# andrewjong/SwapNet

Hardware: AMD Instinct MI355X
Metric: images/sec full G+D step, warp-stage 256x256 bs=32/GPU (higher is better)
Workload: dtype f32; 1 GPU; warp-stage G+D optimize_parameters step, 256x256, bs 32/GPU, fp32 storage and accumulation, GEMM products on the 16-bit MFMA pipe from operand splits: forward / input-gradient GEMMs as 2 fp16 planes of amax-scaled operands (22 of 24 mantissa bits, 3 of 4 terms, the dropped one below 2^-22), weight-gradient GEMMs in the same two-plane form, train mode (dropout 0.5), WarpModule 137.6M + PatchGAN 2.8; step_form=eager launches, global_batch=32, parallelism=dp1

## Files before the change

### include/swapnet_hip.h

```cpp
#ifndef SWAPNET_HIP_H
#define SWAPNET_HIP_H

#include <stddef.h>
#include <stdint.h>

#ifdef __cplusplus
extern "C" {
#endif

typedef struct swn_ctx swn_ctx;
typedef struct swn_model swn_model;

int swn_abi_version(void);
const char* swn_last_error(void);
int swn_is_device_build(void);

int swn_ctx_create(int device, void* hip_stream, int create_stream, size_t workspace_bytes, swn_ctx** out);
int swn_ctx_destroy(swn_ctx* ctx);
int swn_ctx_set_overlap(swn_ctx* ctx, int on);
int swn_ctx_set_patchgan_layers(swn_ctx* ctx, int n_layers);
int swn_ctx_set_patchgan_norm(swn_ctx* ctx, int kind);
int swn_ctx_sync(swn_ctx* ctx);
int swn_ctx_bytes_allocated(swn_ctx* ctx, size_t* out);

int swn_prof_enable(int on);
int swn_prof_reset(void);
int swn_prof_report(char* buf, int len);
int swn_probe_mfma(swn_ctx* ctx, int zeros, int iters, float* out4);
int swn_route_trace(int on);
int swn_route_report(char* buf, int len);
int swn_slot_audit(int on);

int swn_warp_model_create(swn_ctx* ctx, int batch, int height, int width, int is_train, float dropout,
                          swn_model** out);
int swn_texture_model_create(swn_ctx* ctx, int batch, int height, int width, int is_train, int num_roi,
// ... 84 lines not shown
int swn_model_weight_arena(swn_model* m, int net, float** dev_ptr, size_t* count);
int swn_model_arena(swn_model* m, int net, int which, float** dev_ptr, size_t* count);

int swn_op_roi_align(swn_ctx* ctx, const float* tex, int b, int c, int h, int w, const float* rois, int r,
                     int ph, int pw, float* out);
int swn_op_roi_align_indices(swn_ctx* ctx, const float* rois, int k, int h, int w, int ph, int pw, int32_t* idx,
                             uint8_t* valid);
int swn_op_decode_labels(swn_ctx* ctx, const float* x, int b, int c, int h, int w, uint8_t* rgb);
int swn_op_argmax_labels(swn_ctx* ctx, const float* x, int b, int c, int h, int w, int32_t* labels);
int swn_op_labels_to_onehot(swn_ctx* ctx, const int32_t* labels, int b, int c, int h, int w, float* out);
int swn_op_conv(swn_ctx* ctx, int kind, int transposed, int what, int naive, float* x, int n, int ci, int h, int w,
                float* wgt, int co, const float* bias, int act, float* y);
int swn_op_conv_produced(swn_ctx* ctx, int kind, int transposed, int what, int naive, float* x, int n, int ci, int h, int w,
                         float* wgt, int co, const float* bias, int act, float* y, int pre, int post, float* x_out, float* x_slot,
                         float* y_slot, float* z_slot, float* dy_out, float* dy_slot, int* kscale_out);
int swn_op_instance_norm_act(swn_ctx* ctx, const float* x, int n, int c, int h, int w, int act, float* y);
int swn_op_instance_norm_act_bwd(swn_ctx* ctx, const float* x, const float* dy, int n, int c, int h, int w, int act,
                                 float* dx);
int swn_op_batch_norm_act(swn_ctx* ctx, const float* x, int n, int c, int h, int w, int groups, int act, int training,
                          const float* weight, const float* bias, float* running_mean, float* running_var,
                          int64_t* num_batches_tracked, float* y, float* save_stats);
int swn_op_batch_norm_act_bwd(swn_ctx* ctx, const float* x, const float* dy, int n, int c, int h, int w, int groups, int act,
                              const float* weight, const float* bias, float* dx, float* dweight, float* dbias);
int swn_op_batch_norm_act_dropout(swn_ctx* ctx, const float* x, const float* dy, int n, int c, int h, int w, int act, float p,
                                  uint64_t seed, const float* weight, const float* bias, float* y, float* mask, float* dx,
                                  float* dweight, float* dbias);
int swn_op_norm_act_time(swn_ctx* ctx, int kind, int what, const float* x, const float* dy, int n, int c, int h, int w, int groups,
                         int act, int warmup, int iters, float* ms_out);
int swn_op_affine_gather(swn_ctx* ctx, const float* src, float* dst, int b, int c, int h, int w, const double* maps,
                         int nmaps);
// ... 37 lines not shown
```

### swapnet_amd/_C.py

```python
import ctypes as C
import os

_HERE = os.path.dirname(os.path.abspath(__file__))
LIB_PATH = os.path.join(_HERE, "csrc", "libswapnet_hip.so")

LOSS_NAMES = ("D", "D_real", "D_fake", "G", "G_gan", "G_ce", "G_l1", "G_content", "G_style", "D_gp")


class SwnHyper(C.Structure):
    _fields_ = [(n, C.c_float) for n in ("lr", "d_lr", "weight_decay", "d_weight_decay", "b1", "b2",
                                         "lambda_gan", "lambda_ce", "lambda_l1", "lambda_content",
                                         "lambda_style")] + [("gan_mode", C.c_int), ("warp_mode_ce", C.c_int), ("grad_scale", C.c_float),
                                                                           ("d_b1", C.c_float), ("d_b2", C.c_float),
                                                                           ("gp_mode", C.c_int), ("lambda_gp", C.c_float)]


class SwapnetHipError(RuntimeError):
    pass


_vp, _fp, _i, _f = C.c_void_p, C.c_void_p, C.c_int, C.c_float

_PROTOS = {
    "swn_abi_version": ([], _i),
    "swn_is_device_build": ([], _i),
    "swn_ctx_create": ([_i, _vp, _i, C.c_size_t, C.POINTER(_vp)], _i),
    "swn_ctx_destroy": ([_vp], _i),
    "swn_ctx_sync": ([_vp], _i),
    "swn_ctx_set_overlap": ([_vp, _i], _i),
    "swn_ctx_set_patchgan_layers": ([_vp, _i], _i),
    "swn_ctx_set_patchgan_norm": ([_vp, _i], _i),
    "swn_ctx_bytes_allocated": ([_vp, C.POINTER(C.c_size_t)], _i),
    "swn_prof_enable": ([_i], _i),
    "swn_prof_reset": ([], _i),
    "swn_prof_report": ([C.c_char_p, _i], _i),
    "swn_probe_mfma": ([_vp, _i, _i, C.POINTER(C.c_float)], _i),
    "swn_route_trace": ([_i], _i),
    "swn_route_report": ([C.c_char_p, _i], _i),
    "swn_slot_audit": ([_i], _i),
    "swn_warp_model_create": ([_vp, _i, _i, _i, _i, _f, C.POINTER(_vp)], _i),
    "swn_texture_model_create": ([_vp, _i, _i, _i, _i, _i, C.POINTER(_vp)], _i),
    "swn_warp_model_create_ex": ([_vp, _i, _i, _i, _i, _f, _i, _i, C.POINTER(_vp)], _i),
    "swn_texture_model_create_ex": ([_vp, _i, _i, _i, _i, _i, _i, C.POINTER(_vp)], _i),
    "swn_texture_model_create_netG": ([_vp, _i, _i, _i, _i, _i, _i, _i, C.POINTER(_vp)], _i),
    "swn_model_create_shared": ([_vp, _i, _i, _i, C.POINTER(_vp)], _i),
# ... 42 lines not shown
    "swn_model_step": ([_vp, C.POINTER(_f * 3), _i, C.c_uint64], _i),
    "swn_model_step_captured": ([_vp, C.POINTER(_f * 3), _i, C.c_uint64], _i),
    "swn_model_step_dp": ([_vp, C.POINTER(_f * 3), _i, C.c_uint64, _i], _i),
    "swn_ctx_attach_comm": ([_vp, _vp, _vp, _i], _i),
    "swn_model_get_losses": ([_vp, C.POINTER(_f), _i], _i),
    "swn_model_grad_arena": ([_vp, _i, C.POINTER(_vp), C.POINTER(C.c_size_t)], _i),
    "swn_model_weight_arena": ([_vp, _i, C.POINTER(_vp), C.POINTER(C.c_size_t)], _i),
    "swn_model_arena": ([_vp, _i, _i, C.POINTER(_vp), C.POINTER(C.c_size_t)], _i),
    "swn_op_roi_align": ([_vp, _fp, _i, _i, _i, _i, _fp, _i, _i, _i, _fp], _i),
    "swn_op_roi_align_indices": ([_vp, _fp, _i, _i, _i, _i, _i, _vp, _vp], _i),
    "swn_op_decode_labels": ([_vp, _fp, _i, _i, _i, _i, _vp], _i),
    "swn_op_argmax_labels": ([_vp, _fp, _i, _i, _i, _i, _vp], _i),
    "swn_op_labels_to_onehot": ([_vp, _vp, _i, _i, _i, _i, _fp], _i),
    "swn_op_conv": ([_vp, _i, _i, _i, _i, _fp, _i, _i, _i, _i, _fp, _i, _fp, _i, _fp], _i),
    "swn_op_conv_produced": ([_vp, _i, _i, _i, _i, _fp, _i, _i, _i, _i, _fp, _i, _fp, _i, _fp, _i, _i, _fp, _fp, _fp, _fp, _fp, _fp, _vp], _i),
    "swn_op_instance_norm_act": ([_vp, _fp, _i, _i, _i, _i, _i, _fp], _i),
    "swn_op_instance_norm_act_bwd": ([_vp, _fp, _fp, _i, _i, _i, _i, _i, _fp], _i),
    "swn_op_batch_norm_act": ([_vp, _fp, _i, _i, _i, _i, _i, _i, _i, _fp, _fp, _fp, _fp, _vp, _fp, _fp], _i),
    "swn_op_batch_norm_act_bwd": ([_vp, _fp, _fp, _i, _i, _i, _i, _i, _i, _fp, _fp, _fp, _fp, _fp], _i),
    "swn_op_batch_norm_act_dropout": ([_vp, _fp, _fp, _i, _i, _i, _i, _i, _f, C.c_uint64, _fp, _fp, _fp, _fp, _fp, _fp, _fp], _i),
    "swn_op_norm_act_time": ([_vp, _i, _i, _fp, _fp, _i, _i, _i, _i, _i, _i, _i, _i, C.POINTER(C.c_float)], _i),
    "swn_op_affine_gather": ([_vp, _fp, _fp, _i, _i, _i, _i, _vp, _i], _i),
    "swn_op_texture_batch": ([_vp, _vp, _i, _i, _i, _vp, _i, _i, _fp, _i, _fp, C.POINTER(_f), C.POINTER(_f), _i, _i, _i, _i, _i,
                             _fp, _fp, _fp, _fp], _i),
    "swn_op_resize_u8": ([_vp, _vp, C.c_size_t, _vp, _i, _i, _i, _vp], _i),
    "swn_op_warp_batch": ([_vp, _vp, _i, _i, _i, _vp, _vp, _i, _i, _vp, _i, C.POINTER(_f), C.POINTER(_f), _i, _i, _i, _i, _i, _i,
                          _fp, _fp, _fp], _i),
    "swn_op_gan_loss": ([_vp, _i, _fp, _i, _i, _i, _i, _f, _i, _f, _fp, _fp], _i),
    "swn_op_loss": ([_vp, _i, _fp, _fp, _i, _i, _i, _i, _i, _f, _i, _i, _i, _fp, _fp, _fp], _i),
    "swn_op_bias_grad": ([_vp, _fp, _i, _i, _i, _i, _i, _fp], _i),
# ... 67 lines not shown
```

### swapnet_amd/csrc/capi.cpp

```cpp
#include <algorithm>
#include <cstring>
#include <memory>
#include <string>
#include <vector>

#include "../../include/swapnet_hip.h"
#include <cstdlib>

#include "engine.h"

using namespace swn;

struct CtxBox {
  std::unique_ptr<Ctx> c;
  void* owned_stream = nullptr;
  ~CtxBox() { c.reset(); if (owned_stream) stream_destroy(owned_stream); }
};
struct swn_ctx {
  std::shared_ptr<CtxBox> box;
  Ctx* c = nullptr;
};
struct swn_model {
  std::shared_ptr<CtxBox> keep;
  std::shared_ptr<Model> sharer;
// ... 71 lines not shown
    ctx->c->attach_comm(reinterpret_cast<Ctx::AllReduceFn>(fn), comm, fn ? world_size : 1);
  });
}
int swn_ctx_set_patchgan_layers(swn_ctx* ctx, int n_layers) {
  return guard([&] {
    REQUIRE(ctx, "ctx is NULL");
    REQUIRE(n_layers >= 0 && n_layers <= 5, "n_layers_D must be in [1, 5], or 0 for the 1x1 PixelDiscriminator");
    ctx->c->patchgan_layers = n_layers;
  });
}
int swn_ctx_set_patchgan_norm(swn_ctx* ctx, int kind) {
  return guard([&] {
    REQUIRE(ctx, "ctx is NULL");
    REQUIRE(kind >= 0 && kind <= 2, "normalization layer is not found (0 instance, 1 batch, 2 none)");
    ctx->c->patchgan_norm = kind;
  });
}
int swn_ctx_sync(swn_ctx* ctx) {
  return guard([&] { REQUIRE(ctx, "ctx is NULL"); stream_sync(ctx->c->s); });
}
int swn_ctx_bytes_allocated(swn_ctx* ctx, size_t* out) {
  return guard([&] { REQUIRE(ctx && out, "NULL argument"); *out = ctx->c->bytes_allocated; });
}

int swn_prof_enable(int on) { return guard([&] { prof_enable(on); }); }
int swn_prof_reset(void) { return guard([&] { prof_reset(); }); }
int swn_prof_report(char* buf, int len) { return prof_report(buf, len); }
int swn_probe_mfma(swn_ctx* ctx, int zeros, int iters, float* out4) {
  return guard([&] {
    REQUIRE(ctx && out4, "swn_probe_mfma: NULL argument");
// ... 618 lines not shown
        unpack_weight(s, wd.ws, A.g + wd.off, wgt);
      } else {
        A.version += 1;
        net.refresh_dgrad();
        net.backward(false, true);
        nhwc_to_nchw(s, xv.g, x, ci);
      }
      if (dy_out) nhwc_to_nchw(s, yv.g, dy_out, co);
      copy_slot(dy_slot, yv.gbase, "y.g");
    }
    if (kscale_out && net.kscale_n) dev_copy(s, kscale_out, net.kscale, std::min<size_t>(net.kscale_n, 8) * sizeof(int));
    stream_sync(s);
  });
}

int swn_op_instance_norm_act(swn_ctx* ctx, const float* x, int n, int c, int h, int w, int act, float* y) {
  return guard([&] {
    REQUIRE(ctx && x && y && c % 4 == 0, "bad argument (C must be a multiple of 4)");
    Ctx tmp(ctx->c->s);
    ParamArena A; Net net(tmp, A);
    Var xv = net.alloc_var(n, h, w, c, true), yv = net.alloc_var(n, h, w, c, true);
    net.norm_act(xv, yv, true, act, 0.f);
    net.finalize({});
    nchw_to_nhwc(tmp.s, x, n, c, h, w, xv.v);
    net.forward();
    nhwc_to_nchw(tmp.s, yv.v, y, c);
    stream_sync(tmp.s);
  });
}
int swn_op_instance_norm_act_bwd(swn_ctx* ctx, const float* x, const float* dy, int n, int c, int h, int w, int act,
// ... 511 lines not shown
```

### swapnet_amd/csrc/engine.cpp

```cpp
#include "engine.h"
#include <memory>

#include <algorithm>
#include <cstddef>
#include <cstdlib>
#include <cstring>
#include <map>
#include <string>
#include <vector>

namespace swn {

namespace {
int g_route = 0;
std::string g_route_label = "-";
char g_route_phase = '-';
std::vector<std::string> g_route_lines;
std::map<std::string, int> g_route_seen;
}
void route_enable(int on) {
  g_route = on;
  if (on) { g_route_lines.clear(); g_route_seen.clear(); g_route_label = "-"; g_route_phase = '-'; }
}
bool route_on() { return g_route != 0; }
void route_label(const char* label, char phase) { g_route_label = label ? label : "-"; g_route_phase = phase; }
void route_note(const char* kernel) {
  if (!g_route) return;
  std::string line = g_route_label + " " + std::string(1, g_route_phase) + " " + kernel;
  if (g_route_seen.emplace(line, 1).second) g_route_lines.push_back(line);
}
namespace { int g_slot_audit = 0; }
void slot_audit(int on) { g_slot_audit = on; }
bool slot_audit_on() { return g_slot_audit != 0; }

int route_report(char* buf, int len) {
  std::string out;
  for (auto& l : g_route_lines) { out += l; out += "\n"; }
  if (buf && len > 0) { strncpy(buf, out.c_str(), len - 1); buf[len - 1] = 0; }
  return (int)out.size();
}

Ctx::Ctx(void* stream, size_t ws_bytes) {
  s.handle = stream;
  s.ws_bytes = ws_bytes;
  s.ws = static_cast<char*>(dev_alloc(ws_bytes));
}
Ctx::Ctx(const Stream& shared) : s(shared), owns_ws(false) {}
Ctx::~Ctx() {
  try {
    if (owned_comm_stream) stream_sync(comm_stream);
    if (has_side) stream_sync(side);
  } catch (...) {}
  release(allocs);
  if (owns_ws) dev_free(s.ws);
// ... 528 lines not shown
  const bool wslots = wm != 2;
  const size_t slV = wslots ? reserve_slot() : 0, slD = wslots ? reserve_slot() : 0, slX = wslots ? reserve_slot() : 0;
  const bool wgrad_pairs = wslots && conv_wgrad_takes_pairs(wT, Cip, Cop);
  const bool pairV_ok = wslots && wino_fwd_takes_pairs(Cip, Cop) && (!y.has_grad || wgrad_pairs);
  const bool pairD_ok = wslots && wgrad_pairs && (!(wadj && x.has_grad && y.has_grad) || wino_fwd_takes_pairs(Cop, Cip));
  const bool pairX_ok = wslots && wino_fwd_takes_pairs(Cop, Cip);
  const size_t kV = wslots ? reserve_k() : 0, kD = wslots ? reserve_k() : 0, kX = wslots ? reserve_k() : 0;
  float* keepdM = (wadj && y.has_grad && x.has_grad && share_dy()) ? static_cast<float*>(ctx.alloc((size_t)wP * wT * Cop * sizeof(float))) : nullptr;
  const size_t pcw_off = pcw ? reserve_dgp(pcw_bs * wP) : 0, uf_off = pcw ? 0 : reserve_dg(self, (size_t)wP * Cip * Cop);
  wsV_need = std::max(wsV_need, std::max((size_t)wP * wT * std::max(Cip, Cop), (size_t)wP * wT2 * Cop));
  wsM_need = std::max(wsM_need, std::max((size_t)wP * wT * std::max(Cip, Cop), (size_t)wP * wT2 * Cip));
  wsU_need = std::max(wsU_need, (size_t)wP * Cip * Cop);
  const bool y_folds = actf != ACT_NONE && actf != ACT_TANH && wm != 2;
  const size_t ySlot = note_writer(y.vbase, y_folds);
  const float* xbase = x.vbase;
  op.fwd = [=](Net& n) {
    n.need(self);
    float* V = keepV ? keepV : n.wsV;
    const float* xin = pairV_ok ? n.slot_if_complete(xbase) : nullptr;
    wino_input_transform(n.ctx.s, wm, wr, xv, 1, gf.pad_mode, wTh, wTw, V, wslots ? n.amax + slV : nullptr, xin, n.kscale + kV);
    conv_fwd(n.ctx.s, plane_gemm(V, n.wsM, wT, Cip, Cop, Co, wP, plane_scale(xin != nullptr, n.kscale + kV, wslots ? n.amax + slV : nullptr),
                                 {pcw ? nullptr : n.dg + uf_off, n.dgp + pcw_off, pcw, pcw_bs}));
    wino_output_transform(n.ctx.s, wm, wr, n.wsM, Cop, wTh, wTw, bi >= 0 ? A->w + A->params[bi].off : nullptr, actf, yv, Co, 0,
                          y_folds ? n.amax + ySlot : nullptr);
  };

  Var scratch;
  if (y.has_grad && actf != ACT_NONE) scratch = alloc_var(yv.N, yv.H, yv.W, Cop, false);
  const bool want_dx = x.has_grad && y.has_grad;
  const int pcwt = (want_dx && wm != 2) ? wino_precut_tile(Cop, Cip) : 0;
  const size_t pcwt_bs = pcwt ? conv_precut_elems(Cop, Cip, pcwt) : 0;
  size_t pcwt_off = 0, ub_off = 0;
  if (want_dx) {
    if (pcwt) pcwt_off = reserve_dgp(pcwt_bs * wP);
    else ub_off = reserve_dg(self, (size_t)wP * Cop * Cip);
    op.grad_targets.push_back(x);
  }
// ... 360 lines not shown
  const uint64_t salt = ops.size() + 1;
  if (drop_p > 0.f) drop_sites.push_back({salt, raw.v.N, raw.v.H, raw.v.W, raw.v.C, drop_p});
  if (residual && actf != ACT_NONE) throw Error(1, "norm_act: an activation in front of a residual add is not supported");
  note_act(actf, y.v);
  const TView rv = raw.v, rg = raw.g, yv = y.v, yg = y.g;
  const size_t ySlot = note_writer(y.vbase, true);
  const size_t gSlot = (y.has_grad && raw.has_grad) ? note_writer(raw.gbase, true) : 0;
  const bool has_res = residual != nullptr;
  const Var res = has_res ? *residual : Var();
  const double* partial_in = nullptr;
  int partial_chunks = 0;
  if (norm && raw.v.H * raw.v.W > 1024 && raw.v.p == raw.vbase) {
    auto it = conv_stats.find(raw.vbase);
    if (it != conv_stats.end()) { *it->second.use = true; partial_in = it->second.partial; partial_chunks = it->second.chunks; }
  }
  op->fwd = [=](Net& n) {
    NormActArgs a;
    a.x = rv; a.y = yv; a.stats = stats; a.norm = norm; a.act = actf;
    a.partial_in = partial_in; a.partial_chunks = partial_chunks;
    a.drop_p = n.training ? drop_p : 0.f; a.seed = Net::drop_seed(n.seed, salt);
    a.seed_base = n.seed_dev; a.salt = salt;
    a.residual = has_res ? &res.v : nullptr;
    a.amax_out = n.amax + ySlot;
    norm_act_fwd(n.ctx.s, a);
  };
  if (has_res && res.has_grad && y.has_grad) op->grad_targets.push_back(res);
  const bool do_bwd = y.has_grad && raw.has_grad;
  double* colsum = nullptr;
  if (do_bwd && norm && norm_act_bwd_emits_colsum(raw.v.H * raw.v.W, raw.v.C) && raw.g.cs == raw.g.C) {
    colsum = static_cast<double*>(ctx.alloc((size_t)raw.v.N * raw.v.C * sizeof(double)));
    colsums[raw.g.p] = {colsum, raw.v.N};
// ... 779 lines not shown
```

### swapnet_amd/csrc/engine.h

```cpp
#pragma once
#include <cstdlib>
#include <functional>
#include <map>
#include <memory>
#include <string>
#include <vector>

#include "ops.h"

namespace swn {

struct Ctx {
  Stream s;
  Stream side;
  bool has_side = false, side_dirty = false;
  bool side_enabled = true;
  bool use_side() const { return has_side && side_enabled; }
  std::vector<void*> fork_events;
  size_t fork_i = 0;
  void* join_event = nullptr;
  void* owned_side_stream = nullptr;
  void enable_side(int device);
  Stream& fork_side();
  void join_side();
// ... 7 lines not shown
  void* comm_handle = nullptr;
  int comm_world = 1;
  int device_index = 0;
  Stream comm_stream;
  void* owned_comm_stream = nullptr;
  std::vector<void*> comm_events;
  size_t comm_ev_i = 0;
  void* comm_join_event = nullptr;
  bool comm_dirty = false;
  void attach_comm(AllReduceFn fn, void* comm, int world);
  Stream& comm_fork();
  void comm_join();
  void all_reduce_sum(Stream& on, float* buf, size_t count);
  int patchgan_layers = 3;
  int patchgan_norm = 0;
  explicit Ctx(void* stream, size_t ws_bytes);
  explicit Ctx(const Stream& shared);
  bool owns_ws = true;
  ~Ctx();
  void* alloc(size_t bytes);
  Ctx(const Ctx&) = delete;
  Ctx& operator=(const Ctx&) = delete;
};

struct AllocScope {
  Ctx& c; Ctx::AllocList* prev;
  AllocScope(Ctx& ctx, Ctx::AllocList& list) : c(ctx), prev(ctx.sink) { c.sink = &list; }
  ~AllocScope() { c.sink = prev; }
  AllocScope(const AllocScope&) = delete;
  AllocScope& operator=(const AllocScope&) = delete;
// ... 76 lines not shown
  int* kscale = nullptr;
  size_t kscale_n = 0;
  size_t reserve_k() { return kscale_n++; }
  struct BufSlot { size_t off = 0; bool complete = true; };
  std::map<const float*, BufSlot> buf_slots;
  std::map<const float*, const float*> ext_slots;
  size_t note_writer(const float* base, bool folds) {
    auto it = buf_slots.find(base);
    if (it == buf_slots.end()) it = buf_slots.emplace(base, BufSlot{reserve_slot(), true}).first;
    if (!folds) it->second.complete = false;
    else fold_writer_ops.push_back(ops.size());
    return it->second.off;
  }
  struct StatLink { double* partial = nullptr; int chunks = 0; std::shared_ptr<bool> use; };
  std::map<const float*, StatLink> conv_stats;
  std::vector<size_t> fold_writer_ops;
  void set_external_slot(const float* base, const float* slot) { ext_slots[base] = slot; }
  const float* slot_if_complete(const float* base) const {
    auto e = ext_slots.find(base);
    auto it = buf_slots.find(base);
    if (e != ext_slots.end()) return (it == buf_slots.end()) ? e->second : nullptr;
    if (it == buf_slots.end() || !it->second.complete || !amax) return nullptr;
    return amax + it->second.off;
  }
  bool share_dy() const;
  int dg_version = 0;
  bool keep_wino_inputs = false;
  bool s2_wino = true;
  size_t wsV_need = 0, wsM_need = 0, wsU_need = 0;
  float *wsV = nullptr, *wsM = nullptr, *wsU = nullptr;
// ... 254 lines not shown
```

### swapnet_amd/csrc/ops.h

```cpp
#pragma once
#include "common.h"
#include <cmath>
#include <cstdlib>
#include <functional>

namespace swn {

struct WShape;

inline bool env_on(const char* v) { return !(v && atoi(v) == 0); }
inline int env_int(const char* v, int dflt) { return v ? atoi(v) : dflt; }

struct Stream {
  void* handle = nullptr;
  char* ws = nullptr;
  size_t ws_bytes = 0;
};

void* event_create();
void event_destroy(void* ev);
void event_record(void* ev, Stream& s);
void stream_wait_event(Stream& s, void* ev);

void* stream_create_current();
// ... 90 lines not shown
void bias_grad(Stream& s, const TView& dy, float* db);

void reflect_fold(Stream& s, const TView& dxpad, const TView& dx, int accumulate);

void wino_input_transform(Stream& s, int m, int r, const TView& x, int pad, int pad_mode, int Th, int Tw, float* V,
                          float* amax_out = nullptr, const float* in_amax = nullptr, int* kscale_out = nullptr);
void wino_filter_transform(Stream& s, int m, int r, const WShape& w, int mode, const float* packed, float* U);
void wino_filter_transform_pc(Stream& s, int m, int r, const WShape& w, int mode, const float* packed, int bn, uint16_t* out,
                              size_t panel_elems, const float** amax_io = nullptr);
void wino_input_adjoint(Stream& s, int m, int r, float* dV, int C, int pad, int pad_mode, int Th, int Tw, const TView& dx,
                        int accumulate);
void wino_output_transform(Stream& s, int m, int r, const float* M, int Cm, int Th, int Tw, const float* bias, int act,
                           const TView& y, int Cout, int accumulate, float* amax_out = nullptr);
void wino_dy_transform(Stream& s, int m, int r, const TView& dy, int Th, int Tw, float* dM, float* amax_out = nullptr,
                       const float* in_amax = nullptr, int* kscale_out = nullptr);
void tailw_filter_transform(Stream& s, const WShape& w, const float* folded, float* U);
void tailw_filter_grad(Stream& s, const WShape& w, const float* dU, float* dfolded);
void tailw_output_transform(Stream& s, const float* M, int Th, int Tw, int Npad, const float* bias, int act, const TView& y, int Cout);
void tailw_dy_transform(Stream& s, const TView& dy, int Th, int Tw, int Npad, float* dM, float* amax_out = nullptr,
                        const float* in_amax = nullptr, int* kscale_out = nullptr);
void wino_s2_input_transform(Stream& s, const TView& fine, int Th, int Tw, float* V, float* amax_out = nullptr,
                             const float* in_amax = nullptr, int* kscale_out = nullptr);
void wino_s2_input_adjoint(Stream& s, float* dV, int Cf, int Th, int Tw, const TView& fine, const float* bias, int accumulate);
void wino_s2_filter_transform(Stream& s, const WShape& w, int mode, const float* packed, float* U);
void wino_s2_filter_grad(Stream& s, const WShape& w, const float* dU, float* dpacked);
void wino_filter_grad(Stream& s, int m, int r, const WShape& w, const float* dU, float* dpacked);

struct NormActArgs {
  TView x;
  TView y;
// ... 258 lines not shown
```

### swapnet_amd/csrc/wino.hip

```cpp
#include "hip_util.h"

namespace swn {
namespace {

__device__ __forceinline__ float4 f4add(float4 a, float4 b) { return make_float4(a.x + b.x, a.y + b.y, a.z + b.z, a.w + b.w); }
__device__ __forceinline__ float4 f4sub(float4 a, float4 b) { return make_float4(a.x - b.x, a.y - b.y, a.z - b.z, a.w - b.w); }

__device__ __forceinline__ int wsrc(int e, int ext, int pad_mode) {
  if (pad_mode == PAD_REFLECT) {
    if (e < 0) e = -e;
    else if (e >= ext) e = 2 * ext - 2 - e;
    return e;
  }
  return (e < 0 || e >= ext) ? -1 : e;
}

__global__ __launch_bounds__(256) void wino_input_kernel(const float* x, int xcs, int N, int H, int W, int C, int pad,
                                                         int pad_mode, int Th, int Tw, float* V) {
  const int C4 = C >> 2;
  const size_t T = (size_t)N * Th * Tw;
  const size_t total = T * C4;
  for (size_t i = (size_t)blockIdx.x * 256 + threadIdx.x; i < total; i += (size_t)gridDim.x * 256) {
    const size_t tile = i / C4;
    const int c = (int)(i - tile * C4) * 4;
// ... 1020 lines not shown
    }
#pragma unroll
    for (int p = 0; p < A; ++p)
#pragma unroll
      for (int j = 0; j < A; ++j) {
        float4 s = F4ZERO;
#pragma unroll
        for (int jj = 0; jj < M; ++jj) f4mac(s, F43::AT[jj][j], rr[p][jj]);
        *reinterpret_cast<float4*>(dM + ((size_t)(p * A + j) * T + tile) * CM + ph * Npad + c) = pair ? pair4(s, psc) : s;
        am = fmaxf(am, f4amax(s));
      }
  }
  if (!pair) amax_fold(am, amax_out);
}

inline unsigned wgrid(size_t total) { return (unsigned)std::min<size_t>(std::max<size_t>((total + 255) / 256, 1), 256 * 32); }

}

static int variant(int m, int r) {
  if (m == 2 && r == 3) return 0;
  if (m == 4 && r == 3) return 1;
  if (m == 3 && r == 4) return 2;
  if (m == 4 && r == 2) return 3;
  throw Error(1, "winograd: supported forms are F(2,3), F(4,3), F(3,4) and the strided F(4,2)");
}
static constexpr int wino_vec_width() { return 2; }
static float input_gain(int v) { return v == 3 ? 9.f : 100.f; }
static float dy_gain(int v) { return v == 1 ? 225.f : (v == 2 ? 49.f : 16.f); }
void wino_input_transform(Stream& s, int m, int r, const TView& x, int pad, int pad_mode, int Th, int Tw, float* V, float* amax_out,
// ... 56 lines not shown
  const dim3 grid(wgrid(total));
  if (v == 0)
    hipLaunchKernelGGL(wino_output_kernel, grid, dim3(256), 0, hs(s), M, Cm, y.N, Th, Tw, bias, act, y.p, y.cs, y.H, y.W,
                       Cout, accumulate);
  else if (v == 1)
    hipLaunchKernelGGL(winog_output_kernel<F43>, grid, dim3(256), 0, hs(s), M, Cm, y.N, Th, Tw, bias, act, y.p, y.cs, y.H,
                       y.W, Cout, accumulate, amax_out);
  else if (v == 2)
    hipLaunchKernelGGL(winog_output_kernel<F34>, grid, dim3(256), 0, hs(s), M, Cm, y.N, Th, Tw, bias, act, y.p, y.cs, y.H,
                       y.W, Cout, accumulate, amax_out);
  else
    hipLaunchKernelGGL(winog_output_kernel<F42>, grid, dim3(256), 0, hs(s), M, Cm, y.N, Th, Tw, bias, act, y.p, y.cs, y.H,
                       y.W, Cout, accumulate, amax_out);
  check_launch("wino_output_transform");
}
void wino_dy_transform(Stream& s, int m, int r, const TView& dy, int Th, int Tw, float* dM, float* amax_out, const float* in_amax,
                       int* kscale_out) {
  const int v = variant(m, r);
  if (dy.C % 4 || dy.cs % 4) throw Error(1, "wino_dy_transform: C must be a multiple of 4");
  const int vw = v == 0 ? 4 : wino_vec_width();
  const size_t total = (size_t)dy.N * Th * Tw * (dy.C / vw);
  const dim3 grid(wgrid(total));
  if (v == 0 && in_amax) throw Error(1, "wino_dy_transform: F(2,3) planes have no pair form");
#define SWN_WDY_LAUNCH(F, VW)                                                                                                       \
  hipLaunchKernelGGL((winog_dy_kernel<F, VW>), grid, dim3(256), 0, hs(s), dy.p, dy.cs, dy.N, dy.H, dy.W, dy.C, Th, Tw, dM, amax_out, \
                     in_amax, dy_gain(v), kscale_out)
  if (v == 0)
    hipLaunchKernelGGL(wino_dy_kernel, grid, dim3(256), 0, hs(s), dy.p, dy.cs, dy.N, dy.H, dy.W, dy.C, Th, Tw, dM);
  else if (v == 1) SWN_WDY_LAUNCH(F43, 2);
  else if (v == 2) SWN_WDY_LAUNCH(F34, 2);
// ... 101 lines not shown
```

### swapnet_amd/engine.py

```python
import ctypes as C
import os
from collections import OrderedDict

import torch

from . import _C

NET_G, NET_D, NET_VGG = 0, 1, 2
OPT_ADAMW, OPT_ADABOUND = 0, 1
W_WEIGHT, W_GRAD, W_EXP_AVG, W_EXP_AVG_SQ = 0, 1, 2, 3
NORM_KINDS = {"instance": 0, "batch": 1, "none": 2}
NETG_KINDS = {"swapnet": 0, "unet_128": 1}


class Context:

    def __init__(self, device=None, lib=None, workspace_mb=512, use_torch_stream=True):
        self.lib = lib or _C.lib()
        if self.lib.is_device:
            if not torch.cuda.is_available():
                raise _C.SwapnetHipError("no HIP device visible; swapnet_amd has no CPU path")
            self.device = torch.device("cuda", torch.cuda.current_device() if device is None else int(device))
            torch.cuda.set_device(self.device)
            self.torch_stream = torch.cuda.current_stream(self.device)
# ... 36 lines not shown
            cs.wait_event(st["events"][i])
        with torch.cuda.stream(cs):
            buf.copy_(t, non_blocking=True)
        main.wait_stream(cs)
        return buf, (key, i)

    def consumed(self, token):
        if token is None:
            return
        ev = torch.cuda.Event()
        ev.record(torch.cuda.current_stream(self.device))
        self._staging[token[0]]["events"][token[1]] = ev

    def set_overlap(self, on):
        self.lib.call("swn_ctx_set_overlap", self.handle, int(bool(on)))

    def sync(self):
        self.lib.call("swn_ctx_sync", self.handle)

    def attach_comm(self, fn_ptr, comm, world):
        self.lib.call("swn_ctx_attach_comm", self.handle, C.c_void_p(fn_ptr) if fn_ptr else None,
                      comm if comm is not None else None, int(world))

    def route_trace(self, on):
        self.lib.call("swn_route_trace", int(bool(on)))

    def route_report(self):
        need = self.lib.dll.swn_route_report(None, 0)
        buf = C.create_string_buffer(need + 16)
        self.lib.dll.swn_route_report(buf, need + 16)
# ... 766 lines not shown
```

Before: 1342 images/sec.

## Fuse Winograd output transform, instance norm, and next input transform in resblocks

Adds a fused kernel for small (≤16x16) resblock feature maps. One launch does the F(4,3) Winograd output transform, instance-norm statistics, activation, dropout, residual add, and the next conv's Winograd input transform, keeping the tile in shared memory. The graph builder links producer conv → norm → consumer conv through chain links so the separate output-transform, norm and input-transform launches are skipped. This cuts launches and global-memory round trips on the bottleneck layers. The costs are a statically derived amax bound for the pair-scale, low parallelism (grid C/32 × N), and order-sensitive mutable flags in the closures.

Result: no change. 1356 images/sec (median of 6 runs) (+1.0%).

```diff
diff --git a/include/swapnet_hip.h b/include/swapnet_hip.h
--- a/include/swapnet_hip.h
+++ b/include/swapnet_hip.h
@@ -19,6 +19,7 @@
 int swn_ctx_destroy(swn_ctx* ctx);
 int swn_ctx_set_overlap(swn_ctx* ctx, int on);
 int swn_ctx_set_patchgan_layers(swn_ctx* ctx, int n_layers);
+int swn_ctx_set_resblock_chain(swn_ctx* ctx, int on);
 int swn_ctx_set_patchgan_norm(swn_ctx* ctx, int kind);
 int swn_ctx_sync(swn_ctx* ctx);
 int swn_ctx_bytes_allocated(swn_ctx* ctx, size_t* out);
@@ -133,6 +134,9 @@
 int swn_op_conv_produced(swn_ctx* ctx, int kind, int transposed, int what, int naive, float* x, int n, int ci, int h, int w,
                          float* wgt, int co, const float* bias, int act, float* y, int pre, int post, float* x_out, float* x_slot,
                          float* y_slot, float* z_slot, float* dy_out, float* dy_slot, int* kscale_out);
+int swn_op_res_chain(swn_ctx* ctx, const float* x0, int n, int c, int h, int w, const float* w1, const float* b1, const float* w2,
+                     const float* b2, const float* w3, const float* b3, float drop_p, int use_residual, int keep_v, uint64_t seed,
+                     float* raw1, float* h_out, float* raw2, float* rn, float* out, float* stats1, float* stats2, int* kscale_out);
 int swn_op_instance_norm_act(swn_ctx* ctx, const float* x, int n, int c, int h, int w, int act, float* y);
 int swn_op_instance_norm_act_bwd(swn_ctx* ctx, const float* x, const float* dy, int n, int c, int h, int w, int act,
                                  float* dx);
diff --git a/swapnet_amd/_C.py b/swapnet_amd/_C.py
--- a/swapnet_amd/_C.py
+++ b/swapnet_amd/_C.py
@@ -29,6 +29,7 @@
     "swn_ctx_sync": ([_vp], _i),
     "swn_ctx_set_overlap": ([_vp, _i], _i),
     "swn_ctx_set_patchgan_layers": ([_vp, _i], _i),
+    "swn_ctx_set_resblock_chain": ([_vp, _i], _i),
     "swn_ctx_set_patchgan_norm": ([_vp, _i], _i),
     "swn_ctx_bytes_allocated": ([_vp, C.POINTER(C.c_size_t)], _i),
     "swn_prof_enable": ([_i], _i),
@@ -101,6 +102,7 @@
     "swn_op_labels_to_onehot": ([_vp, _vp, _i, _i, _i, _i, _fp], _i),
     "swn_op_conv": ([_vp, _i, _i, _i, _i, _fp, _i, _i, _i, _i, _fp, _i, _fp, _i, _fp], _i),
     "swn_op_conv_produced": ([_vp, _i, _i, _i, _i, _fp, _i, _i, _i, _i, _fp, _i, _fp, _i, _fp, _i, _i, _fp, _fp, _fp, _fp, _fp, _fp, _vp], _i),
+    "swn_op_res_chain": ([_vp, _fp, _i, _i, _i, _i, _fp, _fp, _fp, _fp, _fp, _fp, _f, _i, _i, C.c_uint64, _fp, _fp, _fp, _fp, _fp, _fp, _fp, _vp], _i),
     "swn_op_instance_norm_act": ([_vp, _fp, _i, _i, _i, _i, _i, _fp], _i),
     "swn_op_instance_norm_act_bwd": ([_vp, _fp, _fp, _i, _i, _i, _i, _i, _fp], _i),
     "swn_op_batch_norm_act": ([_vp, _fp, _i, _i, _i, _i, _i, _i, _i, _fp, _fp, _fp, _fp, _vp, _fp, _fp], _i),
diff --git a/swapnet_amd/csrc/capi.cpp b/swapnet_amd/csrc/capi.cpp
--- a/swapnet_amd/csrc/capi.cpp
+++ b/swapnet_amd/csrc/capi.cpp
@@ -109,6 +109,12 @@
     REQUIRE(ctx, "ctx is NULL");
     REQUIRE(kind >= 0 && kind <= 2, "normalization layer is not found (0 instance, 1 batch, 2 none)");
     ctx->c->patchgan_norm = kind;
+  });
+}
+int swn_ctx_set_resblock_chain(swn_ctx* ctx, int on) {
+  return guard([&] {
+    REQUIRE(ctx, "ctx is NULL");
+    ctx->c->resblock_chain = on != 0;
   });
 }
 int swn_ctx_sync(swn_ctx* ctx) {
@@ -757,6 +763,54 @@
   });
 }
 
+int swn_op_res_chain(swn_ctx* ctx, const float* x0, int n, int c, int h, int w, const float* w1, const float* b1, const float* w2,
+                     const float* b2, const float* w3, const float* b3, float drop_p, int use_residual, int keep_v, uint64_t seed,
+                     float* raw1, float* h_out, float* raw2, float* rn, float* out, float* stats1, float* stats2, int* kscale_out) {
+  return guard([&] {
+    const float* wgt[3] = {w1, w2, w3};
+    const float* bias[3] = {b1, b2, b3};
+    REQUIRE(ctx && x0 && w1 && w2 && w3, "NULL argument");
+    REQUIRE(c % 4 == 0 && drop_p >= 0.f && drop_p < 1.f, "bad argument (C must be a multiple of 4, 0 <= p < 1)");
+    Ctx tmp(ctx->c->s);
+    tmp.resblock_chain = ctx->c->resblock_chain;
+    ParamArena A;
+    Net net(tmp, A);
+    net.keep_wino_inputs = keep_v != 0;
+    Var v0 = net.alloc_var(n, h, w, c, false), x = net.alloc_var(n, h, w, c, true);
+    Var r1 = net.alloc_var(n, h, w, c, true), hh = net.alloc_var(n, h, w, c, true), r2 = net.alloc_var(n, h, w, c, true);
+    Var rr = net.alloc_var(n, h, w, c, true), o = net.alloc_var(n, h, w, c, true);
+    net.norm_act(v0, x, true, ACT_RELU, 0.f);
+    net.conv("c1", x, r1, CK_K3S1_REFLECT, c, c, bias[0] != nullptr, ACT_NONE);
+    net.norm_act(r1, hh, true, ACT_RELU, drop_p);
+    float* st1 = net.last_stats;
+    net.conv("c2", hh, r2, CK_K3S1_REFLECT, c, c, bias[1] != nullptr, ACT_NONE);
+    net.norm_act(r2, rr, true, ACT_NONE, 0.f, use_residual ? &x : nullptr);
+    float* st2 = net.last_stats;
+    net.conv("c3", rr, o, CK_K3S1_REFLECT, c, c, bias[2] != nullptr, ACT_NONE);
+    A.allocate(tmp);
+    net.finalize({});
+    Stream& s = tmp.s;
+    const char* names[3] = {"c1", "c2", "c3"};
+    for (int i = 0; i < 3; ++i) {
+      const ParamDesc& wd = A.params[A.index.at(std::string(names[i]) + ".weight")];
+      pack_weight(s, wd.ws, wgt[i], A.w + wd.off);
+      if (bias[i]) dev_copy(s, A.w + A.params[A.index.at(std::string(names[i]) + ".bias")].off, bias[i], c * sizeof(float));
+    }
+    nchw_to_nhwc(s, x0, n, c, h, w, v0.v);
+    net.training = true; net.seed = seed;
+    net.forward();
+    if (raw1) nhwc_to_nchw(s, r1.v, raw1, c);
+    if (h_out) nhwc_to_nchw(s, hh.v, h_out, c);
+    if (raw2) nhwc_to_nchw(s, r2.v, raw2, c);
+    if (rn) nhwc_to_nchw(s, rr.v, rn, c);
+    if (out) nhwc_to_nchw(s, o.v, out, c);
+    if (stats1) dev_copy(s, stats1, st1, (size_t)n * c * 2 * sizeof(float));
+    if (stats2) dev_copy(s, stats2, st2, (size_t)n * c * 2 * sizeof(float));
+    if (kscale_out && net.kscale_n) dev_copy(s, kscale_out, net.kscale, std::min<size_t>(net.kscale_n, 16) * sizeof(int));
+    stream_sync(s);
+  });
+}
+
 int swn_op_instance_norm_act(swn_ctx* ctx, const float* x, int n, int c, int h, int w, int act, float* y) {
   return guard([&] {
     REQUIRE(ctx && x && y && c % 4 == 0, "bad argument (C must be a multiple of 4)");
diff --git a/swapnet_amd/csrc/engine.cpp b/swapnet_amd/csrc/engine.cpp
--- a/swapnet_amd/csrc/engine.cpp
+++ b/swapnet_amd/csrc/engine.cpp
@@ -2,6 +2,7 @@
 #include <memory>
 
 #include <algorithm>
+#include <cmath>
 #include <cstddef>
 #include <cstdlib>
 #include <cstring>
@@ -38,6 +39,30 @@
   for (auto& l : g_route_lines) { out += l; out += "\n"; }
   if (buf && len > 0) { strncpy(buf, out.c_str(), len - 1); buf[len - 1] = 0; }
   return (int)out.size();
+}
+
+__attribute__((weak)) bool wino_res_chain_fits(int H, int W, int C) {
+  return H >= 4 && W >= 4 && H <= 16 && W <= 16 && H % 4 == 0 && W % 4 == 0 && C % 32 == 0;
+}
+__attribute__((weak)) void wino_res_chain(Stream& s, const WinoResChainArgs& a) {
+  if (is_device_build()) throw Error(1, "wino_res_chain: the device library was linked without its kernel");
+  if (!wino_res_chain_fits(a.raw.H, a.raw.W, a.raw.C)) throw Error(1, "wino_res_chain: maps of at most 16x16 (multiples of 4), C a multiple of 32");
+  if (!a.M || !a.stats) throw Error(1, "wino_res_chain: M planes and a stats buffer required");
+  if (a.V && a.pair && (!a.kscale_out || (a.residual && !a.res_amax))) throw Error(1, "wino_res_chain: pair form needs kscale_out and the residual's amax slot");
+  const int Th = a.raw.H / 4, Tw = a.raw.W / 4;
+  wino_output_transform(s, 4, 3, a.M, a.Cm, Th, Tw, a.bias, ACT_NONE, a.raw, a.raw.C, 0, nullptr);
+  NormActArgs na;
+  na.x = a.raw; na.y = a.y; na.stats = a.stats; na.norm = 1; na.act = a.act;
+  na.drop_p = a.drop_p; na.seed = a.seed; na.seed_base = a.seed_base; na.salt = a.salt;
+  na.residual = a.residual; na.amax_out = a.y_amax;
+  norm_act_fwd(s, na);
+  if (!a.V) return;
+  if (!a.pair) { wino_input_transform(s, 4, 3, a.y, 1, PAD_REFLECT, Th, Tw, a.V, a.v_amax, nullptr, a.kscale_out); return; }
+  float bound[AMAX_SLOT] = {0};
+  bound[0] = std::sqrt((float)(a.raw.H * a.raw.W));
+  if (a.drop_p > 0.f) bound[0] *= 1.0f / (1.0f - a.drop_p);
+  if (a.residual) bound[0] += *std::max_element(a.res_amax, a.res_amax + AMAX_SLOT);
+  wino_input_transform(s, 4, 3, a.y, 1, PAD_REFLECT, Th, Tw, a.V, nullptr, bound, a.kscale_out);
 }
 
 Ctx::Ctx(void* stream, size_t ws_bytes) {
@@ -596,13 +621,31 @@
   const bool y_folds = actf != ACT_NONE && actf != ACT_TANH && wm != 2;
   const size_t ySlot = note_writer(y.vbase, y_folds);
   const float* xbase = x.vbase;
+  std::shared_ptr<ChainLink> cin;
+  if (wm == 4 && wr == 3 && kind == CK_K3S1_REFLECT && x.v.p == x.vbase && x.v.cs == Cip) {
+    auto it = chain_outputs.find(x.vbase);
+    if (it != chain_outputs.end() && !it->second->has_consumer && it->second->norm_op + 1 == ops.size()) {
+      cin = it->second;
+      cin->has_consumer = true; cin->keepV = keepV; cin->slV = slV; cin->kV = kV; cin->pairV_ok = pairV_ok; cin->xbase = xbase;
+    }
+  }
+  std::shared_ptr<ChainLink> cprod;
+  if (ctx.resblock_chain && wm == 4 && wr == 3 && actf == ACT_NONE && Co == Cop && wino_res_chain_fits(y.v.H, y.v.W, Cop) &&
+      y.v.p == y.vbase && y.v.cs == Cop) {
+    cprod = std::make_shared<ChainLink>();
+    cprod->producer_op = ops.size(); cprod->A = A; cprod->bi = bi; cprod->Cm = Cop; cprod->producer = L.name;
+    chain_offers[y.vbase] = cprod;
+  }
   op.fwd = [=](Net& n) {
     n.need(self);
     float* V = keepV ? keepV : n.wsV;
     const float* xin = pairV_ok ? n.slot_if_complete(xbase) : nullptr;
-    wino_input_transform(n.ctx.s, wm, wr, xv, 1, gf.pad_mode, wTh, wTw, V, wslots ? n.amax + slV : nullptr, xin, n.kscale + kV);
+    const bool have_v = cin && cin->v_fresh;
+    if (cin) cin->v_fresh = false;
+    if (!have_v) wino_input_transform(n.ctx.s, wm, wr, xv, 1, gf.pad_mode, wTh, wTw, V, wslots ? n.amax + slV : nullptr, xin, n.kscale + kV);
     conv_fwd(n.ctx.s, plane_gemm(V, n.wsM, wT, Cip, Cop, Co, wP, plane_scale(xin != nullptr, n.kscale + kV, wslots ? n.amax + slV : nullptr),
                                  {pcw ? nullptr : n.dg + uf_off, n.dgp + pcw_off, pcw, pcw_bs}));
+    if (cprod && cprod->taken) { cprod->m_fresh = true; return; }
     wino_output_transform(n.ctx.s, wm, wr, n.wsM, Cop, wTh, wTw, bi >= 0 ? A->w + A->params[bi].off : nullptr, actf, yv, Co, 0,
                           y_folds ? n.amax + ySlot : nullptr);
   };
@@ -993,7 +1036,37 @@
     auto it = conv_stats.find(raw.vbase);
     if (it != conv_stats.end()) { *it->second.use = true; partial_in = it->second.partial; partial_chunks = it->second.chunks; }
   }
+  std::shared_ptr<ChainLink> link;
+  if (norm && raw.v.p == raw.vbase && raw.v.cs == raw.v.C && raw.v.H * raw.v.W <= 256 && raw.v.C % 32 == 0) {
+    auto it = chain_offers.find(raw.vbase);
+    if (it != chain_offers.end() && !it->second->taken && it->second->producer_op + 1 == ops.size()) {
+      link = it->second;
+      link->taken = true; link->norm_op = ops.size();
+      chain_outputs[y.vbase] = link;
+    }
+  }
+  const float* resbase = has_res ? res.vbase : nullptr;
   op->fwd = [=](Net& n) {
+    if (link && link->m_fresh) {
+      link->m_fresh = false;
+      WinoResChainArgs c;
+      c.M = n.wsM; c.Cm = link->Cm; c.bias = link->bi >= 0 ? link->A->w + link->A->params[link->bi].off : nullptr;
+      c.raw = rv; c.y = yv; c.stats = stats; c.act = actf;
+      c.drop_p = n.training ? drop_p : 0.f; c.seed = Net::drop_seed(n.seed, salt); c.seed_base = n.seed_dev; c.salt = salt;
+      c.residual = has_res ? &res.v : nullptr;
+      c.y_amax = n.amax + ySlot;
+      const bool pair = link->has_consumer && link->pairV_ok && n.slot_if_complete(link->xbase) != nullptr;
+      const float* rslot = (pair && has_res) ? n.slot_if_complete(resbase) : nullptr;
+      const bool with_v = link->has_consumer && !(pair && has_res && !rslot);
+      if (with_v) {
+        c.V = link->keepV ? link->keepV : n.wsV;
+        c.v_amax = n.amax + link->slV; c.pair = pair ? 1 : 0; c.kscale_out = n.kscale + link->kV; c.res_amax = rslot;
+        link->v_fresh = true;
+      }
+      if (route_on()) route_note(("wino_res_chain[" + link->producer + (with_v ? (pair ? ": full, V pair]" : ": full, V fp32]") : ": tail]")).c_str());
+      wino_res_chain(n.ctx.s, c);
+      return;
+    }
     NormActArgs a;
     a.x = rv; a.y = yv; a.stats = stats; a.norm = norm; a.act = actf;
     a.partial_in = partial_in; a.partial_chunks = partial_chunks;
diff --git a/swapnet_amd/csrc/engine.h b/swapnet_amd/csrc/engine.h
--- a/swapnet_amd/csrc/engine.h
+++ b/swapnet_amd/csrc/engine.h
@@ -45,6 +45,7 @@
   void all_reduce_sum(Stream& on, float* buf, size_t count);
   int patchgan_layers = 3;
   int patchgan_norm = 0;
+  int resblock_chain = 1;
   explicit Ctx(void* stream, size_t ws_bytes);
   explicit Ctx(const Stream& shared);
   bool owns_ws = true;
@@ -151,6 +152,18 @@
   }
   struct StatLink { double* partial = nullptr; int chunks = 0; std::shared_ptr<bool> use; };
   std::map<const float*, StatLink> conv_stats;
+  struct ChainLink {
+    size_t producer_op = 0, norm_op = 0;
+    std::string producer;
+    ParamArena* A = nullptr; int bi = -1;
+    int Cm = 0;
+    bool taken = false;
+    bool m_fresh = false;
+    bool has_consumer = false;
+    float* keepV = nullptr; size_t slV = 0, kV = 0; bool pairV_ok = false; const float* xbase = nullptr;
+    bool v_fresh = false;
+  };
+  std::map<const float*, std::shared_ptr<ChainLink>> chain_offers, chain_outputs;
   std::vector<size_t> fold_writer_ops;
   void set_external_slot(const float* base, const float* slot) { ext_slots[base] = slot; }
   const float* slot_if_complete(const float* base) const {
diff --git a/swapnet_amd/csrc/ops.h b/swapnet_amd/csrc/ops.h
--- a/swapnet_amd/csrc/ops.h
+++ b/swapnet_amd/csrc/ops.h
@@ -128,6 +128,22 @@
                            const TView& y, int Cout, int accumulate, float* amax_out = nullptr);
 void wino_dy_transform(Stream& s, int m, int r, const TView& dy, int Th, int Tw, float* dM, float* amax_out = nullptr,
                        const float* in_amax = nullptr, int* kscale_out = nullptr);
+struct WinoResChainArgs {
+  const float* M = nullptr; int Cm = 0;
+  const float* bias = nullptr;
+  TView raw, y;
+  const TView* residual = nullptr;
+  const float* res_amax = nullptr;
+  float* stats = nullptr;
+  int act = ACT_NONE;
+  float drop_p = 0.f; uint64_t seed = 0; const uint64_t* seed_base = nullptr; uint64_t salt = 0;
+  float* y_amax = nullptr;
+  float* V = nullptr;
+  float* v_amax = nullptr;
+  int pair = 0; int* kscale_out = nullptr;
+};
+bool wino_res_chain_fits(int H, int W, int C);
+void wino_res_chain(Stream& s, const WinoResChainArgs& a);
 void tailw_filter_transform(Stream& s, const WShape& w, const float* folded, float* U);
 void tailw_filter_grad(Stream& s, const WShape& w, const float* dU, float* dfolded);
 void tailw_output_transform(Stream& s, const float* M, int Th, int Tw, int Npad, const float* bias, int act, const TView& y, int Cout);
diff --git a/swapnet_amd/csrc/wino.hip b/swapnet_amd/csrc/wino.hip
--- a/swapnet_amd/csrc/wino.hip
+++ b/swapnet_amd/csrc/wino.hip
@@ -1058,6 +1058,189 @@
   if (!pair) amax_fold(am, amax_out);
 }
 
+struct ResChainP {
+  const float* M; int Cm; const float* bias;
+  float* raw; int rcs; float* y; int ycs; const float* res; int rescs;
+  float* stats;
+  int N, H, W, C, act;
+  float drop_p; uint64_t seed; const uint64_t* seed_base; uint64_t salt;
+  float* y_amax;
+  float* V; float* v_amax; const float* res_amax; int pair; int* kscale_out;
+};
+
+template <bool XFORM>
+__global__ __launch_bounds__(256, 4) void wino_res_chain_kernel(ResChainP p) {
+  typedef F43 F;
+  typedef fvec<2> vt;
+  constexpr int A = 6, M = 4;
+  __shared__ float slab[16 * 16 * 32];
+  double* red = reinterpret_cast<double*>(slab);
+  float* x0s = slab + 2048;
+  const uint64_t drop_seed_v = p.seed_base ? *p.seed_base * 0x9E3779B1ull + p.salt : p.seed;
+  const int t = threadIdx.x, cp = t & 15, tl = t >> 4;
+  const int Tw = p.W >> 2, nt = (p.H >> 2) * Tw, HW = p.H * p.W;
+  const int n = blockIdx.y, c = blockIdx.x * 32 + cp * 2;
+  const bool live = tl < nt;
+  const int tq = live ? tl : nt - 1;
+  const int ty = tq / Tw, tx = tq - ty * Tw;
+  const size_t T = (size_t)p.N * nt;
+  const unsigned tile = (unsigned)(n * nt + tq), moff = tile * (unsigned)p.Cm + c, voff = tile * (unsigned)p.C + c;
+
+  vt o[M][M];
+  {
+    vt m[A][A];
+#pragma unroll
+    for (int a = 0; a < A; ++a)
+#pragma unroll
+      for (int b = 0; b < A; ++b) m[a][b] = *reinterpret_cast<const vt*>(p.M + (size_t)(a * A + b) * T * p.Cm + moff);
+    vt s1[M][A];
+#pragma unroll
+    for (int b = 0; b < A; ++b)
+#pragma unroll
+      for (int r = 0; r < M; ++r) {
+        vt s = vt(0.f);
+#pragma unroll
+        for (int k = 0; k < A; ++k)
+          if (F::AT[r][k] != 0.f) s += F::AT[r][k] * m[k][b];
+        s1[r][b] = s;
+      }
+    vt bv = vt(0.f);
+    if (p.bias) bv = *reinterpret_cast<const vt*>(p.bias + c);
+#pragma unroll
+    for (int a = 0; a < M; ++a)
+#pragma unroll
+      for (int b = 0; b < M; ++b) {
+        vt v = vt(0.f);
+#pragma unroll
+        for (int k = 0; k < A; ++k)
+          if (F::AT[b][k] != 0.f) v += F::AT[b][k] * s1[a][k];
+        o[a][b] = v + bv;
+      }
+  }
+  if (live) {
+#pragma unroll
+    for (int a = 0; a < M; ++a)
+#pragma unroll
+      for (int b = 0; b < M; ++b)
+        *reinterpret_cast<vt*>(p.raw + ((size_t)(n * p.H + M * ty + a) * p.W + M * tx + b) * p.rcs + c) = o[a][b];
+  }
+
+  if (tl == 0) { x0s[cp * 2] = o[0][0][0]; x0s[cp * 2 + 1] = o[0][0][1]; }
+  __syncthreads();
+  const double x00 = (double)x0s[cp * 2], x01 = (double)x0s[cp * 2 + 1];
+  double s[4] = {0, 0, 0, 0};
+  const double kk = live ? 1.0 : 0.0;
+#pragma unroll
+  for (int a = 0; a < M; ++a)
+#pragma unroll
+    for (int b = 0; b < M; ++b) {
+      const double a0 = ((double)o[a][b][0] - x00) * kk, a1 = ((double)o[a][b][1] - x01) * kk;
+      s[0] += a0; s[1] += a1; s[2] += a0 * a0; s[3] += a1 * a1;
+    }
+#pragma unroll
+  for (int j = 0; j < 4; ++j) red[(tl * 16 + cp) * 4 + j] = s[j];
+  __syncthreads();
+#pragma unroll
+  for (int stride = 8; stride >= 1; stride >>= 1) {
+    if (tl < stride) {
+#pragma unroll
+      for (int j = 0; j < 4; ++j) red[(tl * 16 + cp) * 4 + j] += red[((tl + stride) * 16 + cp) * 4 + j];
+    }
+    __syncthreads();
+  }
+  float mean[2], rstd[2];
+#pragma unroll
+  for (int j = 0; j < 2; ++j) {
+    const double md = red[cp * 4 + j] / HW;
+    double var = red[cp * 4 + 2 + j] / HW - md * md;
+    if (var < 0) var = 0;
+    mean[j] = (float)((j ? x01 : x00) + md); rstd[j] = (float)(1.0 / sqrt(var + (double)1e-5f));
+  }
+  if (tl == 0) *reinterpret_cast<float4*>(p.stats + ((size_t)n * p.C + c) * 2) = make_float4(mean[0], rstd[0], mean[1], rstd[1]);
+  __syncthreads();
+
+  float am = 0.f;
+  if (live) {
+#pragma unroll
+    for (int a = 0; a < M; ++a)
+#pragma unroll
+      for (int b = 0; b < M; ++b) {
+        const int pix = (M * ty + a) * p.W + M * tx + b;
+        const size_t e = (size_t)n * HW + pix;
+        vt v;
+#pragma unroll
+        for (int j = 0; j < 2; ++j) {
+          float q = act_apply((o[a][b][j] - mean[j]) * rstd[j], p.act);
+          if (p.drop_p > 0.f) q *= drop_scale(drop_seed_v, e * p.C + c + j, p.drop_p);
+          v[j] = q;
+        }
+        if (p.res) v += *reinterpret_cast<const vt*>(p.res + e * p.rescs + c);
+        *reinterpret_cast<vt*>(p.y + e * p.ycs + c) = v;
+        if (XFORM) *reinterpret_cast<vt*>(slab + pix * 32 + cp * 2) = v;
+        am = fmaxf(am, fvamax<2>(v));
+      }
+  }
+  amax_fold(am, p.y_amax);
+  if (!XFORM) return;
+  __syncthreads();
+
+  float psc = 1.f;
+  if (p.pair) {
+    float rm = 0.f;
+    if (p.res_amax) {
+      const int lane = t & 63;
+      rm = fmaxf(fmaxf(p.res_amax[lane], p.res_amax[lane + 64]), fmaxf(p.res_amax[lane + 128], p.res_amax[lane + 192]));
+#pragma unroll
+      for (int of = 32; of; of >>= 1) rm = fmaxf(rm, __shfl_xor(rm, of));
+    }
+    float bound = sqrtf((float)HW);
+    if (p.drop_p > 0.f) bound *= 1.0f / (1.0f - p.drop_p);
+    const float mm = (bound + rm) * 100.f;
+    int k = 0;
+    if (mm > 0.f && mm <= 3.0e38f) {
+      const int ex = (int)((__float_as_uint(mm) >> 23) & 255u) - 127;
+      k = 14 - ex;
+      k = k < -100 ? -100 : (k > 100 ? 100 : k);
+    }
+    if (p.kscale_out && blockIdx.x == 0 && blockIdx.y == 0 && t == 0) *p.kscale_out = k;
+    psc = __uint_as_float((unsigned)(127 + k) << 23);
+  }
+  int sy[A];
+#pragma unroll
+  for (int a = 0; a < A; ++a) sy[a] = wsrc(M * ty - 1 + a, p.H, PAD_REFLECT);
+  vt tt[A][A];
+#pragma unroll
+  for (int b = 0; b < A; ++b) {
+    const int sx = wsrc(M * tx - 1 + b, p.W, PAD_REFLECT);
+    vt d[A];
+#pragma unroll
+    for (int a = 0; a < A; ++a) d[a] = *reinterpret_cast<const vt*>(slab + (sy[a] * p.W + sx) * 32 + cp * 2);
+#pragma unroll
+    for (int r = 0; r < A; ++r) {
+      vt sm = vt(0.f);
+#pragma unroll
+      for (int k = 0; k < A; ++k)
+        if (F::BT[r][k] != 0.f) sm += F::BT[r][k] * d[k];
+      tt[r][b] = sm;
+    }
+  }
+  float amv = 0.f;
+#pragma unroll
+  for (int a = 0; a < A; ++a)
+#pragma unroll
+    for (int j = 0; j < A; ++j) {
+      vt sm = vt(0.f);
+#pragma unroll
+      for (int k = 0; k < A; ++k)
+        if (F::BT[j][k] != 0.f) sm += F::BT[j][k] * tt[a][k];
+      if (live) {
+        *reinterpret_cast<vt*>(p.V + (size_t)(a * A + j) * T * p.C + voff) = p.pair ? pairv<2>(sm, psc) : sm;
+        amv = fmaxf(amv, fvamax<2>(sm));
+      }
+    }
+  if (!p.pair) amax_fold(amv, p.v_amax);
+}
+
 inline unsigned wgrid(size_t total) { return (unsigned)std::min<size_t>(std::max<size_t>((total + 255) / 256, 1), 256 * 32); }
 
 }
@@ -1144,6 +1327,31 @@
                        y.W, Cout, accumulate, amax_out);
   check_launch("wino_output_transform");
 }
+bool wino_res_chain_fits(int H, int W, int C) { return H >= 4 && W >= 4 && H <= 16 && W <= 16 && H % 4 == 0 && W % 4 == 0 && C % 32 == 0; }
+void wino_res_chain(Stream& s, const WinoResChainArgs& a) {
+  if (!wino_res_chain_fits(a.raw.H, a.raw.W, a.raw.C)) throw Error(1, "wino_res_chain: maps of at most 16x16 (multiples of 4), C a multiple of 32");
+  if ((size_t)a.raw.N * (a.raw.H / 4) * (a.raw.W / 4) * std::max(a.Cm, a.raw.C) >= ((size_t)1 << 31)) throw Error(1, "wino_res_chain: plane too large");
+  if (!a.M || !a.stats || a.Cm % 2 || a.Cm < a.raw.C) throw Error(1, "wino_res_chain: M planes and a stats buffer required");
+  if (a.y.N != a.raw.N || a.y.H != a.raw.H || a.y.W != a.raw.W || a.y.C != a.raw.C) throw Error(1, "wino_res_chain: raw and y differ in shape");
+  if (a.raw.cs % 2 || a.y.cs % 2 || ((uintptr_t)a.raw.p & 7) || ((uintptr_t)a.y.p & 7)) throw Error(1, "wino_res_chain: views not 8-byte tileable");
+  if (a.residual && (a.residual->pixels() != a.raw.pixels() || a.residual->C != a.raw.C || a.residual->cs % 2 || ((uintptr_t)a.residual->p & 7)))
+    throw Error(1, "wino_res_chain: bad residual view");
+  if (a.V && a.pair && (!a.kscale_out || (a.residual && !a.res_amax))) throw Error(1, "wino_res_chain: pair form needs kscale_out and the residual's amax slot");
+  ResChainP p{};
+  p.M = a.M; p.Cm = a.Cm; p.bias = a.bias;
+  p.raw = a.raw.p; p.rcs = a.raw.cs; p.y = a.y.p; p.ycs = a.y.cs;
+  p.res = a.residual ? a.residual->p : nullptr; p.rescs = a.residual ? a.residual->cs : 0;
+  p.stats = a.stats; p.N = a.raw.N; p.H = a.raw.H; p.W = a.raw.W; p.C = a.raw.C; p.act = a.act;
+  p.drop_p = a.drop_p; p.seed = a.seed; p.seed_base = a.seed_base; p.salt = a.salt;
+  p.y_amax = a.y_amax;
+  p.V = a.V; p.v_amax = a.v_amax; p.res_amax = a.residual ? a.res_amax : nullptr; p.pair = a.pair; p.kscale_out = a.kscale_out;
+  const dim3 grid(p.C / 32, p.N);
+  if (a.V) hipLaunchKernelGGL(wino_res_chain_kernel<true>, grid, dim3(256), 0, hs(s), p);
+  else hipLaunchKernelGGL(wino_res_chain_kernel<false>, grid, dim3(256), 0, hs(s), p);
+  check_launch("wino_res_chain");
+  if (a.V && a.pair && slot_audit_on())
+    audit_pair_planes(s, "wino_res_chain", a.V, (size_t)36 * p.N * (p.H / 4) * (p.W / 4) * p.C, a.kscale_out);
+}
 void wino_dy_transform(Stream& s, int m, int r, const TView& dy, int Th, int Tw, float* dM, float* amax_out, const float* in_amax,
                        int* kscale_out) {
   const int v = variant(m, r);
diff --git a/swapnet_amd/engine.py b/swapnet_amd/engine.py
--- a/swapnet_amd/engine.py
+++ b/swapnet_amd/engine.py
@@ -74,6 +74,9 @@
 
     def set_overlap(self, on):
         self.lib.call("swn_ctx_set_overlap", self.handle, int(bool(on)))
+
+    def set_resblock_chain(self, on):
+        self.lib.call("swn_ctx_set_resblock_chain", self.handle, int(bool(on)))
 
     def sync(self):
         self.lib.call("swn_ctx_sync", self.handle)
```
